# 959AI994/Multi-Gate-VAE

Measured on AMD Instinct MI355X. Metric: circuit-graphs/sec (train step), AIG-64k batch=64 per GPU, higher is better.
Workload: dtype f32 storage; dense products as bf16x3 split-precision MFMA, fp32 accumulate; 1 GPU; cfg2: DG_AE --type aig, 64 x 65536-node synthetic levelised DAGs per GPU (N=4194304, E=6558720, 120 levels), H=64, 4+4 rounds, layernorm, weights [1,4,4], negatives sampled; step includes the 7-scalar metrics copy (pinned, read one step behind); global_batch=64, parallelism=dp1

## Files before the change

### include/mgvae_hip.h

```cpp
#ifndef MGVAE_HIP_H
#define MGVAE_HIP_H
#include <stdint.h>
#ifdef __cplusplus
extern "C" {
#endif

#ifndef MGV_OK
#define MGV_OK 0
#define MGV_EINVAL (-1)
#define MGV_EUNSUPPORTED (-2)
#endif

int mgv_abi_version(void);

int mgv_struct_stage_fwd(int H, int64_t N, const float* h_in, const int32_t* nbr_ptr, const int32_t* nbr_idx,
                         const uint8_t* xcls, const float* xtab, int C, const float* Wc, const float* bc,
                         const float* Whh, const float* bhh, const float* ln_w, const float* ln_b, float ln_eps,
                         float* h_out, void* stream);
int mgv_struct_stage_bwd(int H, int64_t N, const float* h_in, const int32_t* nbr_ptr, const int32_t* nbr_idx,
                         const uint8_t* xcls, const float* xtab, int C, const float* Wc, const float* WcT,
                         const float* bc, const float* Whh, const float* WhhT, const float* bhh,
                         const float* ln_w, const float* ln_b, float ln_eps, const float* gy_direct,
                         const float* gy_agg, float* g_direct_out, float* g_agg_out, float* dWc, float* dbc,
                         float* dWhh, float* dbhh, float* dxtab, float* dln_w, float* dln_b, void* stream);
// ... 151 lines not shown
int mgv_cc_class_ws_ints(int64_t N);
int mgv_cc_class_count(int64_t N, const int32_t* label, int min_size, const int32_t* status, int32_t* ws, int64_t ws_ints, int32_t* counts,
                       void* stream);
int mgv_cc_class_fill(int64_t N, const int32_t* label, int64_t C, int64_t M, int32_t* ws, int64_t ws_ints, void* sort_temp,
                      int64_t sort_temp_ints, int64_t* class_ptr, int32_t* members, void* stream);
int mgv_sim_union(int H, int64_t N, const float* y, int ldy, const int32_t* graph_ptr, int G, float threshold, int32_t* parent,
                  int32_t* status, void* stream);
int mgv_recon_loss_fwd(int H, const float* s, const float* t, int ld, const int64_t* pos_src, const int64_t* pos_dst,
                       int64_t Epos, const int64_t* neg_src, const int64_t* neg_dst, int64_t Eneg,
                       double* sums, uint64_t* counts, int32_t* pred_bin, double* workspace, int64_t workspace_doubles,
                       void* stream);
int mgv_recon_loss_bwd(int H, int64_t N, const float* s, const float* t, int ld, const int64_t* pos_src, const int64_t* pos_dst,
                       int64_t Epos, const int32_t* pos_out_ptr, const int32_t* pos_out_dst, const int32_t* pos_in_ptr,
                       const int32_t* pos_in_src, const int64_t* neg_src, const int64_t* neg_dst, int64_t Eneg,
                       const float* gscale, float* ds, float* dt, void* stream);
int mgv_recon_loss_bwd_csr(int H, int64_t N, const float* s, const float* t, int ld, const int32_t* pos_out_ptr,
                           const int32_t* pos_out_dst, const int32_t* pos_in_ptr, const int32_t* pos_in_src, int64_t Epos,
                           const int32_t* neg_out_ptr, const int32_t* neg_out_dst, const int32_t* neg_in_ptr,
                           const int32_t* neg_in_src, int64_t Eneg, const float* gscale, float* ds, float* dt,
                           int skip_pos_longer_than , void* stream);
int mgv_recon_heavy_lists(int H, const float* s, const float* t, int ld, int64_t Epos, const float* gscale, int K,
                          const int32_t* nodes, const int32_t* node_seg_ptr, int S, const int32_t* seg_node, const int32_t* seg_e0,
                          const int32_t* seg_e1, const int32_t* list, int which, float* partial_ws, float* out, void* stream);
int mgv_link_keys(int H, const float* s, const float* t, int ld, const int64_t* pos_src, const int64_t* pos_dst, int64_t P,
                  const int64_t* neg_src, const int64_t* neg_dst, int64_t Q, uint32_t* keys, float* scores, int32_t* status,
                  void* stream);
int mgv_link_rank_work_ints(int64_t n);
int mgv_link_rank(int64_t n, int64_t P, const uint32_t* sorted_keys, const int32_t* order, double* out, int32_t* work,
                  int64_t work_ints, void* stream);
int mgv_neg_sample(int64_t N, int64_t E, uint64_t seed, const int32_t* pos_out_ptr, const int32_t* pos_out_dst,
                   int64_t* neg_src, int64_t* neg_dst, int32_t* cnt_out, int32_t* cnt_in, int32_t* rank_out, int32_t* rank_in,
                   void* stream);
int mgv_neg_bucket(int64_t E, const int64_t* neg_src, const int64_t* neg_dst, const int32_t* out_ptr, const int32_t* in_ptr,
                   const int32_t* rank_out, const int32_t* rank_in, int64_t* srt_src, int64_t* srt_dst, int32_t* out_dst, int32_t* in_src,
                   void* stream);

int mgv_func_loss_fwd(int H, int64_t P, const float* hf, const int64_t* pair_a, const int64_t* pair_b,
                      const float* tt, float eps, float* dis, double* ws, double* workspace, int64_t workspace_doubles,
                      void* stream);
int mgv_func_loss_bwd_csr(int H, int64_t N, int64_t P, const float* hf, const int64_t* pair_a, const int64_t* pair_b, const float* tt_sim,
                          const float* dis, float eps, const double* workspace8, const float* grad_loss, const int32_t* a_ptr,
                          const int32_t* a_pair, const int32_t* b_ptr, const int32_t* b_pair, const float* add, float* dhf, void* stream);
int mgv_func_loss_bwd(int H, int64_t P, const float* hf, const int64_t* pair_a, const int64_t* pair_b,
                      const float* tt, const float* dis, float eps, const double* ws, const float* gscale,
                      float* dhf, void* stream);

// ... 97 lines not shown
```

### multi-gate-vae_amd/csrc/losses.hip

```cpp
#include "mgv_common.h"
#include "mgv_slab.h"
#include "../../include/mgvae_hip.h"

namespace mgv {

__device__ __forceinline__ void atomic_add4(float* p, const float4& v) {
    atomicAdd(p + 0, v.x); atomicAdd(p + 1, v.y); atomicAdd(p + 2, v.z); atomicAdd(p + 3, v.w);
}

__device__ __forceinline__ double block_sum_d(double v, double* red) {
    const int tid = threadIdx.x;
    __syncthreads();
    red[tid] = v;
    __syncthreads();
    for (int s = kThreads / 2; s > 0; s >>= 1) {
        if (tid < s) red[tid] += red[tid + s];
        __syncthreads();
    }
    return red[0];
}

template <int H, bool BWD>
__global__ __launch_bounds__(kThreads) void k_edge_dot(int64_t E, const float* s, const float* t, int ld,
                                                       const int64_t* src, const int64_t* dst, int sigmoid,
                                                       float* out, const float* gout, float* ds, float* dt) {
    constexpr int LPR = H / 4, EPB = kThreads / LPR;
    const int lr = threadIdx.x % LPR, slot = threadIdx.x / LPR;
    for (int64_t e0 = (int64_t)blockIdx.x * EPB; e0 < E; e0 += (int64_t)gridDim.x * EPB) {
        const int64_t e = e0 + slot;
        const bool ok = e < E;
// ... 27 lines not shown
template <int H, bool BWD>
__global__ __launch_bounds__(kThreads) void k_recon(ReconArgs a) {
    constexpr int LPR = H / 4, EPB = kThreads / LPR;
    __shared__ double red[kThreads];
    const int lr = threadIdx.x % LPR, slot = threadIdx.x / LPR;
    const int64_t E = a.Ep + a.En;
    float lp = 0.f, ln = 0.f;
    unsigned int tp = 0, fp = 0, tn = 0, fn = 0;
    float g = 0.f;
    if (BWD) g = *a.gscale;
    const float wpos = BWD ? g / (float)a.Ep : 0.f, wneg = BWD ? g / (float)a.En : 0.f;
    for (int64_t e0 = (int64_t)blockIdx.x * EPB; e0 < E; e0 += (int64_t)gridDim.x * EPB) {
        const int64_t e = e0 + slot;
        const bool ok = e < E;
        const bool pos = e < a.Ep;
        float4 x = zero4(), y = zero4();
        int64_t u = 0, v = 0;
        if (ok) {
            u = pos ? a.psrc[e] : a.nsrc[e - a.Ep];
            v = pos ? a.pdst[e] : a.ndst[e - a.Ep];
            x = ld4(a.s + u * a.ld + 4 * lr);
            y = ld4(a.t + v * a.ld + 4 * lr);
        }
        const float val = group_sum<LPR>(dot4(x, y));
        const float p = sigmoidf_(val);
        if (!BWD) {
            if (ok && lr == 0) {
                const bool hit = p > 0.5f;
                if (pos) { lp -= logf(p + 1e-15f); tp += hit; fn += !hit; }
                else     { ln -= logf((1.0f - p) + 1e-15f); fp += hit; tn += !hit; }
                if (a.pred_bin) a.pred_bin[e] = hit ? 1 : 0;
            }
        } else if (ok) {
            const float dp = p * (1.0f - p);
            const float c = pos ? -wpos * dp / (p + 1e-15f) : wneg * dp / ((1.0f - p) + 1e-15f);
            atomic_add4(a.ds + u * a.ld + 4 * lr, scale4(c, y));
            atomic_add4(a.dt + v * a.ld + 4 * lr, scale4(c, x));
        }
    }
    if (!BWD) {
        const double sp = block_sum_d((double)lp, red);
        const double sn = block_sum_d((double)ln, red);
        const double c0 = block_sum_d((double)tp, red), c1 = block_sum_d((double)fp, red);
        const double c2 = block_sum_d((double)tn, red), c3 = block_sum_d((double)fn, red);
        if (threadIdx.x == 0) {
            a.slab[2 * blockIdx.x + 0] = sp; a.slab[2 * blockIdx.x + 1] = sn;
            atomicAdd(a.cnt + 0, (unsigned long long)c0); atomicAdd(a.cnt + 1, (unsigned long long)c1);
// ... 12 lines not shown
    const float w = -(*gscale) / (float)Ep;
    for (int64_t n0 = (int64_t)blockIdx.x * RPB; n0 < N; n0 += (int64_t)gridDim.x * RPB) {
        const int64_t u = n0 + slot;
        if (u >= N) continue;
        const float4 su = ld4(s + u * ld + 4 * lr), tu = ld4(t + u * ld + 4 * lr);
        float4 gs = zero4(), gt = zero4();
        for (int e = out_ptr[u]; e < out_ptr[u + 1]; ++e) {
            const float4 tv = ld4(t + (int64_t)out_dst[e] * ld + 4 * lr);
            const float p = sigmoidf_(group_sum<LPR>(dot4(su, tv)));
            gs = fma4(w * p * (1.0f - p) / (p + 1e-15f), tv, gs);
        }
        for (int e = in_ptr[u]; e < in_ptr[u + 1]; ++e) {
            const float4 sv = ld4(s + (int64_t)in_src[e] * ld + 4 * lr);
            const float p = sigmoidf_(group_sum<LPR>(dot4(sv, tu)));
            gt = fma4(w * p * (1.0f - p) / (p + 1e-15f), sv, gt);
        }
        float* pds = ds + u * ld + 4 * lr;
        float* pdt = dt + u * ld + 4 * lr;
        st4(pds, add4(ld4(pds), gs));
        st4(pdt, add4(ld4(pdt), gt));
    }
}

template <int H>
__global__ __launch_bounds__(kThreads) void k_recon_bwd_pull2(int64_t N, const float* s, const float* t, int ld,
                                                              const int32_t* pout_ptr, const int32_t* pout_dst, const int32_t* pin_ptr,
                                                              const int32_t* pin_src, int64_t Ep, const int32_t* nout_ptr,
                                                              const int32_t* nout_dst, const int32_t* nin_ptr, const int32_t* nin_src,
                                                              int64_t En, const float* gscale, float* ds, float* dt, int skip_len) {
    constexpr int LPR = H / 4, RPB = kThreads / LPR, K = 4;
    const int lr = threadIdx.x % LPR, slot = threadIdx.x / LPR;
    const float wp = Ep > 0 ? -(*gscale) / (float)Ep : 0.f, wn = En > 0 ? (*gscale) / (float)En : 0.f;
    int64_t first, end, stride;
    if ((gridDim.x & 7) == 0) {
        const int64_t chunk = ((N + 8 * RPB - 1) / (8 * RPB)) * RPB;
        first = (blockIdx.x & 7) * chunk + (int64_t)(blockIdx.x >> 3) * RPB;
        end = min(N, ((blockIdx.x & 7) + 1) * chunk);
        stride = (int64_t)(gridDim.x >> 3) * RPB;
    } else {
        first = (int64_t)blockIdx.x * RPB; end = N; stride = (int64_t)gridDim.x * RPB;
    }
    for (int64_t n0 = first; n0 < end; n0 += stride) {
        const int64_t u = n0 + slot;
        if (u >= end) continue;
        const float4 su = ld4(s + u * ld + 4 * lr), tu = ld4(t + u * ld + 4 * lr);
        int b0 = 0, b1 = 0, b2 = 0, b3 = 0, c0 = 0, c1 = 0, c2 = 0, c3 = 0;
        if (Ep > 0) {
            b0 = pout_ptr[u]; c0 = pout_ptr[u + 1] - b0;
            b1 = pin_ptr[u]; c1 = pin_ptr[u + 1] - b1;
            if (skip_len > 0 && c0 > skip_len) c0 = 0;
            if (skip_len > 0 && c1 > skip_len) c1 = 0;
        }
        if (En > 0) {
            b2 = nout_ptr[u]; c2 = nout_ptr[u + 1] - b2;
            b3 = nin_ptr[u]; c3 = nin_ptr[u + 1] - b3;
// ... 5 lines not shown
        float4 gs = zero4(), gt = zero4();
        int id[K];
#pragma unroll
        for (int k = 0; k < K; ++k) id[k] = k < c3 ? partner(k) : 0;
        for (int j0 = 0; j0 < c3; j0 += K) {
            float4 v[K];
#pragma unroll
            for (int k = 0; k < K; ++k) {
                const int j = j0 + k;
                const bool from_t = j < c0 || (j >= c1 && j < c2);
                if (j < c3) v[k] = ld4((from_t ? t : s) + (int64_t)id[k] * ld + 4 * lr);
            }
            int nid[K];
#pragma unroll
            for (int k = 0; k < K; ++k) nid[k] = j0 + K + k < c3 ? partner(j0 + K + k) : 0;
#pragma unroll
            for (int k = 0; k < K; ++k) {
                const int j = j0 + k;
                if (j < c3) {
                    const bool out = j < c0 || (j >= c1 && j < c2), pos = j < c1;
                    const float p = sigmoidf_(group_sum<LPR>(dot4(out ? su : tu, v[k])));
                    const float c = pos ? wp * p * (1.0f - p) / (p + 1e-15f) : wn * p * (1.0f - p) / ((1.0f - p) + 1e-15f);
                    if (out) gs = fma4(c, v[k], gs); else gt = fma4(c, v[k], gt);
                }
            }
#pragma unroll
            for (int k = 0; k < K; ++k) id[k] = nid[k];
        }
        st4(ds + u * ld + 4 * lr, gs);
        st4(dt + u * ld + 4 * lr, gt);
    }
}

template <int H>
__global__ __launch_bounds__(256) void k_recon_heavy_seg(int S, const int32_t* seg_node, const int32_t* seg_e0, const int32_t* seg_e1,
                                                         const int32_t* nodes, const float* s, const float* t, int ld, const int32_t* list,
                                                         int which, int64_t Ep, const float* gscale, float* partial) {
    constexpr int LPR = H / 4, G = 256 / LPR;
    __shared__ __attribute__((aligned(16))) float s_p[G][H];
    const int lr = threadIdx.x % LPR, grp = threadIdx.x / LPR;
    const float wp = -(*gscale) / (float)Ep;
    for (int sg = blockIdx.x; sg < S; sg += gridDim.x) {
        const int64_t u = nodes[seg_node[sg]];
        const float4 own = ld4((which ? t : s) + u * ld + 4 * lr);
        const float* other = which ? s : t;
        float4 acc = zero4();
        for (int e = seg_e0[sg] + grp; e < seg_e1[sg]; e += G) {
            const float4 v = ld4(other + (int64_t)list[e] * ld + 4 * lr);
            const float p = sigmoidf_(group_sum<LPR>(dot4(own, v)));
            acc = fma4(wp * p * (1.0f - p) / (p + 1e-15f), v, acc);
        }
        __syncthreads();
        st4(&s_p[grp][4 * lr], acc);
        __syncthreads();
        if (grp == 0) {
            float4 tot = zero4();
            for (int g = 0; g < G; ++g) tot = add4(tot, ld4(&s_p[g][4 * lr]));
            st4(partial + (int64_t)sg * H + 4 * lr, tot);
        }
    }
}

template <int H>
__global__ __launch_bounds__(kThreads) void k_recon_bwd_rows(int64_t E, const float* s, const float* t, int ld, const int64_t* src,
                                                             const int64_t* dst, int negative, float wscale, const float* gscale,
                                                             float* ds, float* dt) {
    constexpr int EPB = kThreads / H;
    const int l = threadIdx.x % H, slot = threadIdx.x / H;
    const float w = (*gscale) * wscale;
    for (int64_t e0 = (int64_t)blockIdx.x * EPB; e0 < E; e0 += (int64_t)gridDim.x * EPB) {
        const int64_t e = e0 + slot;
        const bool ok = e < E;
        int64_t u = 0, v = 0;
        float x = 0.f, y = 0.f;
        if (ok) { u = src[e]; v = dst[e]; x = s[u * ld + l]; y = t[v * ld + l]; }
        const float p = sigmoidf_(group_sum<H>(x * y));
        if (!ok) continue;
        const float dp = p * (1.0f - p);
        const float c = negative ? w * dp / ((1.0f - p) + 1e-15f) : -w * dp / (p + 1e-15f);
        atomicAdd(ds + u * ld + l, c * y);
        atomicAdd(dt + v * ld + l, c * x);
    }
}
// ... 254 lines not shown
        const int64_t* es = neg ? neg_src : pos_src;
        const int64_t* ed = neg ? neg_dst : pos_dst;
        const float wsc = 1.0f / (float)E;
        switch (H) {
            case 16: hipLaunchKernelGGL((mgv::k_recon_bwd_rows<16>), dim3(mgv::items_grid(E, mgv::kThreads / 16)), dim3(mgv::kThreads), 0, st, E, s, t, ld, es, ed, neg, wsc, gscale, ds, dt); break;
            case 32: hipLaunchKernelGGL((mgv::k_recon_bwd_rows<32>), dim3(mgv::items_grid(E, mgv::kThreads / 32)), dim3(mgv::kThreads), 0, st, E, s, t, ld, es, ed, neg, wsc, gscale, ds, dt); break;
            case 64: hipLaunchKernelGGL((mgv::k_recon_bwd_rows<64>), dim3(mgv::items_grid(E, mgv::kThreads / 64)), dim3(mgv::kThreads), 0, st, E, s, t, ld, es, ed, neg, wsc, gscale, ds, dt); break;
            default: return MGV_EUNSUPPORTED;
        }
    }
    MGV_LAUNCH_RET();
}

extern "C" int mgv_recon_loss_bwd_csr(int H, int64_t N, const float* s, const float* t, int ld, const int32_t* pos_out_ptr,
                                      const int32_t* pos_out_dst, const int32_t* pos_in_ptr, const int32_t* pos_in_src, int64_t Epos,
                                      const int32_t* neg_out_ptr, const int32_t* neg_out_dst, const int32_t* neg_in_ptr,
                                      const int32_t* neg_in_src, int64_t Eneg, const float* gscale, float* ds, float* dt,
                                      int skip_pos_longer_than, void* stream) {
    MGV_CHECK_ARG(s && t && gscale && ds && dt && Epos >= 0 && Eneg >= 0 && N >= 0 && ld >= H && ld % 4 == 0 && skip_pos_longer_than >= 0);
    MGV_CHECK_ARG(Epos == 0 || (pos_out_ptr && pos_out_dst && pos_in_ptr && pos_in_src));
    MGV_CHECK_ARG(Eneg == 0 || (neg_out_ptr && neg_out_dst && neg_in_ptr && neg_in_src));
    if (N == 0) return MGV_OK;
    hipStream_t st = static_cast<hipStream_t>(stream);
    MGV_DISPATCH_H(H, hipLaunchKernelGGL((mgv::k_recon_bwd_pull2<HH>), dim3(mgv::items_grid(N, mgv::kThreads / (HH / 4))), dim3(mgv::kThreads), 0, st,
                                         N, s, t, ld, pos_out_ptr, pos_out_dst, pos_in_ptr, pos_in_src, Epos, neg_out_ptr, neg_out_dst,
                                         neg_in_ptr, neg_in_src, Eneg, gscale, ds, dt, skip_pos_longer_than));
    MGV_LAUNCH_RET();
}

extern "C" int mgv_recon_heavy_lists(int H, const float* s, const float* t, int ld, int64_t Epos, const float* gscale, int K,
                                     const int32_t* nodes, const int32_t* node_seg_ptr, int S, const int32_t* seg_node, const int32_t* seg_e0,
                                     const int32_t* seg_e1, const int32_t* list, int which, float* partial_ws, float* out, void* stream) {
    MGV_CHECK_ARG(K >= 0 && S >= 0 && Epos > 0 && s && t && gscale && out && ld >= H && ld % 4 == 0 && (which == 0 || which == 1));
    if (K == 0 || S == 0) return MGV_OK;
    MGV_CHECK_ARG(nodes && node_seg_ptr && seg_node && seg_e0 && seg_e1 && list && partial_ws);
    hipStream_t st = static_cast<hipStream_t>(stream);
    MGV_DISPATCH_H(H, hipLaunchKernelGGL((mgv::k_recon_heavy_seg<HH>), dim3(S < 4096 ? S : 4096), dim3(256), 0, st, S, seg_node, seg_e0, seg_e1, nodes,
                                         s, t, ld, list, which, Epos, gscale, partial_ws));
    hipLaunchKernelGGL(mgv::k_heavy_add, dim3((K + 15) / 16 < 1024 ? (K + 15) / 16 : 1024), dim3(256), 0, st, K, H, nodes, node_seg_ptr, partial_ws, out, ld, 1);
    MGV_LAUNCH_RET();
}

extern "C" int mgv_func_loss_fwd(int H, int64_t P, const float* hf, const int64_t* pair_a, const int64_t* pair_b,
                                 const float* tt, float eps, float* dis, double* ws, double* workspace, int64_t workspace_doubles,
                                 void* stream) {
    MGV_CHECK_ARG(P >= 2 && hf && pair_a && pair_b && tt && dis && ws);
    hipStream_t st = static_cast<hipStream_t>(stream);
    int g1 = 0;
    MGV_DISPATCH_H(H, g1 = mgv::items_grid(P, mgv::kThreads / (HH / 4)));
    const int g2 = mgv::items_grid(P, mgv::kThreads);
    MGV_CHECK_ARG(workspace && workspace_doubles >= 4 * (int64_t)g1 && workspace_doubles >= 3 * (int64_t)g2);
    MGV_DISPATCH_H(H, hipLaunchKernelGGL((mgv::k_func_dist<HH>), dim3(g1), dim3(mgv::kThreads), 0, st, P, hf, pair_a, pair_b, tt, eps, dis, workspace));
    mgv::launch_slab_sum<double, double>(workspace, g1, 4, 4, ws, st);
    hipLaunchKernelGGL(mgv::k_func_l1, dim3(g2), dim3(mgv::kThreads), 0, st, P, dis, tt, ws, workspace);
    mgv::launch_slab_sum<double, double>(workspace, g2, 3, 3, ws + 4, st);
    MGV_LAUNCH_RET();
}

extern "C" int mgv_func_loss_bwd_csr(int H, int64_t N, int64_t P, const float* hf, const int64_t* pair_a, const int64_t* pair_b, const float* tt,
                                     const float* dis, float eps, const double* ws, const float* gscale, const int32_t* a_ptr,
                                     const int32_t* a_pair, const int32_t* b_ptr, const int32_t* b_pair, const float* add, float* dhf, void* stream) {
    MGV_CHECK_ARG(N >= 0 && P >= 2 && hf && pair_a && pair_b && tt && dis && ws && gscale && a_ptr && a_pair && b_ptr && b_pair && dhf);
// ... 52 lines not shown
```

### multi-gate-vae_amd/deepgate/_model_base.py

```python
import os

import torch
from torch import nn

from . import ops
from .arch.mlp import MLP
from .arch.tfmlp import TFMlpAggr
from .data import plan_of
from .digae_layer import DirectedInnerProductDecoder
from .sampling import NegativeEdges, negative_sampling, negative_sampling_device

EPS = 1e-15
DEVICE_SAMPLER = True
MAX_LOGSTD = 10


class FunctionalModel(nn.Module):
    ENCODER_ATTR = 'struct_encoder'
    GATES = ()

    def __init__(self, struct_encoder, num_rounds=1, dim_hidden=128, enable_encode=True, enable_reverse=True):
        super().__init__()
        setattr(self, self.ENCODER_ATTR, struct_encoder)
        self.decoder = DirectedInnerProductDecoder()
# ... 100 lines not shown
        with torch.no_grad():
            s, t = self._decoder_halves(hs)
            return ops.reconstruct_edges(s, t, graph_ptr=graph_ptr, threshold=threshold, skip_self=skip_self, by=by,
                                         with_scores=with_scores, max_edges=max_edges)

    def similar_gates(self, hf, k, graph_ptr=None, threshold=0.999):
        return ops.sim_topk(hf, k, graph_ptr=graph_ptr, threshold=threshold)

    def equivalence_candidates(self, hf, graph_ptr=None, threshold=0.999, with_scores=False, max_pairs=None):
        return ops.sim_pairs(hf, graph_ptr=graph_ptr, threshold=threshold, with_scores=with_scores, max_pairs=max_pairs)

    def equivalence_classes(self, hf, graph_ptr=None, threshold=0.999, min_size=2):
        return ops.sim_classes(hf, graph_ptr=graph_ptr, threshold=threshold, min_size=min_size)

    def similarity_profile(self, hf, thresholds, graph_ptr=None):
        return ops.counts_above(ops.sim_profile(hf, thresholds, graph_ptr=graph_ptr))

    def equivalence_threshold(self, hf, max_pairs, graph_ptr=None, lo=0.0):
        return ops.sim_threshold_for(hf, max_pairs, graph_ptr=graph_ptr, lo=lo)

    def functional_similarity(self, hf, pair_index):
        return ops.sim_at(hf, pair_index)

    def recon_loss(self, hs, pos_edge_index, neg_edge_index=None, want_pred=True, edge_keys=None, plan=None, pass_hs=False, want_rank=False):
        if pass_hs and hs.requires_grad:
            st, self._hs_pass = ops.linear_passthrough(hs, self.hs_decompose.weight, self.hs_decompose.bias)
        else:
            st = ops.linear(hs, self.hs_decompose.weight, self.hs_decompose.bias)
        if plan is not None and (plan.E != pos_edge_index.shape[1] or plan.N != hs.shape[0]):
            plan = None
        neg_csr = None
        if neg_edge_index is None:
            neg_edge_index = self._draw_negatives(hs, pos_edge_index, plan, edge_keys)
        if plan is not None and hs.is_cuda and torch.is_tensor(neg_edge_index) and neg_edge_index.shape[1] > 0:
            cache = getattr(plan, '_neg_cache', None)
            key = (neg_edge_index.data_ptr(), neg_edge_index._version, tuple(neg_edge_index.shape), hs.shape[0])
            if cache is None or cache[0] is not neg_edge_index or cache[1] != key:
                from .sampling import bucket_negatives
                cache = plan._neg_cache = (neg_edge_index, key, bucket_negatives(neg_edge_index.long(), hs.shape[0]))
            neg_edge_index = cache[2]
        if isinstance(neg_edge_index, NegativeEdges):
            neg_csr, neg_edge_index = neg_edge_index.csr, neg_edge_index.edge_index
        loss, counts, pred_bin = ops.ReconLossFn.apply(st, pos_edge_index, neg_edge_index, want_pred, plan, neg_csr)
        self.last_confusion = counts
        self.last_link_metrics = ops.link_record(st, None, pos_edge_index, neg_edge_index) if want_rank else None
        Ep, En = pos_edge_index.shape[1], neg_edge_index.shape[1]
        gt_bin = None
        if want_pred:
            gt_bin = torch.zeros(Ep + En, dtype=torch.int32, device=hs.device)
            gt_bin[:Ep] = 1
        return loss, pred_bin if want_pred else None, gt_bin

    def load(self, model_path):
        checkpoint = torch.load(model_path, map_location=lambda storage, loc: storage)
        src = checkpoint['state_dict']
        state = {}
        for k, v in src.items():
            state[k[7:] if k.startswith('module') and not k.startswith('module_list') else k] = v
        own = self.state_dict()
        for k in list(state):
            if k in own:
                if state[k].shape != own[k].shape:
                    print('Skip loading parameter {}, required shape{}, loaded shape{}.'.format(k, own[k].shape, state[k].shape))
                    state[k] = own[k]
            else:
                print('Drop parameter {}.'.format(k))
# ... 11 lines not shown
```

### multi-gate-vae_amd/deepgate/ops.py

```python
from collections import namedtuple

import torch

from . import _hip
from ._hip import HipLibraryError, check, ptr

import os

F32 = torch.float32
I32 = torch.int32
U8 = torch.uint8
LN_EPS = 1e-5

PRECISION = os.environ.get('MGV_PRECISION', 'x3')
FIRST_STAGE_TABLE = True


def use_x3(H):
    return PRECISION == 'x3' and H in (32, 64)


def split_bf16(w):
    hi = w.to(torch.bfloat16)
    lo = (w - hi.to(torch.float32)).to(torch.bfloat16)
    return hi, lo


def frag_order(w):
    R, K = w.shape
    return w.reshape(R // 16, 16, K // 32, 4, 8).permute(0, 2, 3, 1, 4).reshape(-1)
# ... 1360 lines not shown

def sim_classes(x, graph_ptr=None, threshold=SIM_THRESHOLD, min_size=2, route='walk', eps=1e-8, max_pairs=None):
    if route not in ('walk', 'pairs'):
        raise HipLibraryError("sim_classes: route must be 'walk' (classes straight from the tile walk) or 'pairs' (sim_pairs, then "
                              "components), got %r" % (route,))
    min_size = _min_size(min_size)
    if route == 'walk' and max_pairs is not None:
        raise HipLibraryError("sim_classes: max_pairs belongs to route='pairs'; the walk holds no pair list")
    if route == 'pairs':
        pi, _, _ = sim_pairs(x, graph_ptr=graph_ptr, threshold=threshold, max_pairs=max_pairs, eps=eps)
        with torch.no_grad():
            label, status = _cc_from_pairs(pi, x.shape[0])
            return (label,) + _class_table(label, min_size, status, 'sim_classes')
    y = row_unit(x, eps)
    with torch.no_grad():
        N, H = y.shape
        gp, G = _pair_graphs(graph_ptr, y.device)
        parent, status = _cc_forest(N, y.device)
        _hip.call('mgv_sim_union', H, N, ptr(y), H, ptr(gp), G, float(threshold), ptr(parent), ptr(status))
        label = _cc_labels(N, parent)
        return (label,) + _class_table(label, min_size, status, 'sim_classes')


class ReconLossFn(torch.autograd.Function):

    @staticmethod
    def forward(ctx, st, pos_edge_index, neg_edge_index, want_pred, plan=None, neg_csr=None):
        std = check(st.detach().contiguous(), F32, 'st')
        N, H2 = std.shape
        H = H2 // 2
        ps, pd = _edge_rows(pos_edge_index)
        ns, nd = _edge_rows(neg_edge_index)
        Ep, En = ps.numel(), ns.numel()
        dev = std.device
        sums = torch.zeros(2, dtype=torch.float64, device=dev)
        counts = torch.zeros(4, dtype=torch.int64, device=dev)
        pred = torch.empty(Ep + En, dtype=torch.int32, device=dev) if want_pred else None
        t_view = std[:, H:]
        _hip.call('mgv_recon_loss_fwd', H, ptr(std), ptr(t_view), H2, ptr(ps), ptr(pd), Ep, ptr(ns), ptr(nd), En,
                  ptr(sums), ptr(counts), ptr(pred), *_sw(std.device))
        loss = (sums[0] / max(Ep, 1) + sums[1] / max(En, 1)).to(F32)
        ctx.save_for_backward(std, ps, pd, ns, nd)
        ctx.plan, ctx.neg_csr = plan, neg_csr
        ctx.mark_non_differentiable(counts)
        if pred is not None:
            ctx.mark_non_differentiable(pred)
            return loss, counts, pred
        return loss, counts, torch.empty(0, dtype=torch.int32, device=dev)

    @staticmethod
    def backward(ctx, gloss, _gc, _gp):
        global _SWEEP_BWD_EVENT
        if _SWEEP_BWD_EVENT is not None and gloss.is_cuda:
            torch.cuda.current_stream().wait_event(_SWEEP_BWD_EVENT)
            _SWEEP_BWD_EVENT = None
        std, ps, pd, ns, nd = ctx.saved_tensors
        H2 = std.shape[1]
        H = H2 // 2
        g = gloss.detach().to(F32).reshape(1).contiguous()
        pl = ctx.plan
        if pl is not None and ctx.neg_csr is not None:
            dst_ = torch.empty_like(std)
            heavy = [(0, pl.heavy_segments(True), pl.out_dst), (1, pl.heavy_segments(False), pl.in_src)]
            skip = pl.HEAVY_ROW if any(hv is not None for _, hv, _ in heavy) else 0
            _hip.call('mgv_recon_loss_bwd_csr', H, std.shape[0], ptr(std), ptr(std[:, H:]), H2, ptr(pl.out_ptr), ptr(pl.out_dst),
                      ptr(pl.in_ptr), ptr(pl.in_src), ps.numel(), *[ptr(c) for c in ctx.neg_csr], ns.numel(), ptr(g), ptr(dst_),
                      ptr(dst_[:, H:]), skip)
            for which, hv, lst in heavy:
                if hv is not None:
                    pw = workspace(hv['S'] * H, std.device)
                    _hip.call('mgv_recon_heavy_lists', H, ptr(std), ptr(std[:, H:]), H2, ps.numel(), ptr(g), hv['K'], ptr(hv['nodes']),
                              ptr(hv['node_seg_ptr']), hv['S'], ptr(hv['seg_node']), ptr(hv['seg_e0']), ptr(hv['seg_e1']), ptr(lst), which,
                              ptr(pw), ptr(dst_[:, H:]) if which else ptr(dst_))
            return dst_, None, None, None, None, None
        dst_ = torch.zeros_like(std)
        csr = (pl.out_ptr, pl.out_dst, pl.in_ptr, pl.in_src) if pl is not None else (None, None, None, None)
        _hip.call('mgv_recon_loss_bwd', H, std.shape[0], ptr(std), ptr(std[:, H:]), H2, ptr(ps), ptr(pd), ps.numel(),
                  *[ptr(c) for c in csr], ptr(ns), ptr(nd), ns.numel(), ptr(g), ptr(dst_), ptr(dst_[:, H:]))
        return dst_, None, None, None, None, None


def confusion_counts(pred_bin, gt_bin):
    counts = torch.zeros(4, dtype=torch.int64, device=pred_bin.device)
    _hip.call('mgv_confusion', pred_bin.numel(), ptr(check(pred_bin.contiguous(), torch.int32, 'pred_bin')),
              ptr(check(gt_bin.contiguous(), torch.int32, 'gt_bin')), ptr(counts))
    return counts


LINK_RECORD_WORDS = 8


def link_record(st_or_s, t=None, pos_edge_index=None, neg_edge_index=None, return_scores=False):
    neg = getattr(neg_edge_index, 'edge_index', neg_edge_index)
    P, Q = int(pos_edge_index.shape[1]), int(neg.shape[1])
    if P == 0 or Q == 0:
        raise ValueError('Only one class present (%d positive, %d negative pairs): ROC-AUC and average precision are not defined' % (P, Q))
    sd = check(st_or_s.detach().contiguous(), F32, 'st' if t is None else 's')
    if t is None:
        ld = sd.shape[1]
        H = ld // 2
        td = sd[:, H:]
    else:
# ... 293 lines not shown
```

### multi-gate-vae_amd/deepgate/trainer.py

```python
import inspect
import os
import sys
import time

import numpy as np
import torch
from torch import nn

from . import ops
from .data import CircuitBatch
from .optim import FlatAdam
from .prefetch import BatchPrefetcher
from .sampling import sorted_edge_keys
from .synthetic import collate as collate_arrays
from .utils.logger import Logger
from .utils.model_utils import load_model
from .utils.utils import AverageMeter


class GraphLoader:

    def __init__(self, graphs, batch_size, shuffle, rank=0, world_size=1, seed=0):
        self.graphs, self.batch_size, self.shuffle = graphs, batch_size, shuffle
        self.rank, self.world_size, self.seed, self.epoch = rank, world_size, seed, 0
# ... 106 lines not shown
        checkpoint = torch.load(path, map_location='cpu')
        self.optimizer.load_state_dict(checkpoint['optimizer'])
        for param_group in self.optimizer.param_groups:
            self.lr = param_group['lr']
        self.model_epoch = checkpoint['epoch']
        self.model.load(path)
        print('[INFO] Continue training from epoch {:}'.format(self.model_epoch))
        return path

    def resume(self):
        model_path = os.path.join(self.log_dir, 'model_last.pth')
        if os.path.exists(model_path):
            self.model, self.optimizer, self.model_epoch = load_model(self.model, model_path, optimizer=self.optimizer,
                                                                      local_rank=self.local_rank, device=self.device)
            return True
        return False

    def run_batch(self, batch, want_pred=True, want_rank=False):
        batch.train_pos_edge_index = batch.edge_index
        neg = getattr(batch, 'neg_edge_index', None)
        dev_is_cuda = next(self.model.parameters()).is_cuda
        if getattr(self, '_has_after_hs', None) is None:
            self._has_after_hs = 'after_hs' in inspect.signature(self.model.forward).parameters
        side = self._side_stream() if (self.overlap and dev_is_cuda and self._has_after_hs) else None

        def recon(hs, pass_hs=False):
            k = None
            if neg is None and getattr(batch, '_mgv_plan', None) is None:
                k = getattr(batch, '_mgv_edge_keys', None)
                if k is None:
                    k = batch._mgv_edge_keys = sorted_edge_keys(batch.edge_index, batch.num_nodes)
            return self.model.recon_loss(hs, batch.train_pos_edge_index, neg, want_pred=want_pred, edge_keys=k,
                                         plan=getattr(batch, '_mgv_plan', None), **({'pass_hs': True} if pass_hs else {}),
                                         **({'want_rank': True} if want_rank else {}))

        def recon_on_side(hs):
            side.wait_event(self.model._hs_ready)
            hs.record_stream(side)
            with torch.cuda.stream(side):
                return recon(hs, pass_hs=True)

        if side is not None:
            hs, hf = self.model(batch, after_hs=recon_on_side)
            loss, pred_bin, gt_bin = self.model.after_hs_out
            self.model.after_hs_out = None
            main = torch.cuda.current_stream()
            main.wait_stream(side)
            for t in (loss, pred_bin, gt_bin, self.model.last_confusion, self.model.last_link_metrics if want_rank else None):
                if t is not None:
                    t.record_stream(main)
        else:
            hs, hf = self.model(batch)
            loss, pred_bin, gt_bin = recon(hs)
        loss_status = {'recon_loss': loss, 'pred_bin': pred_bin, 'gt_bin': gt_bin}
        if 'VAE' in getattr(self.args, 'model', '') and hasattr(self.model, 'kl_loss'):
            s_kl, t_kl = self.model.kl_loss()
            loss_status['kl_loss'] = s_kl + t_kl
# ... 131 lines not shown
```

Measured before the change: 1007 graphs/s.

## Fuse recon loss forward into backward CSR pull pass with expected grad scale

When a CSR plan and negative CSR are available and predictions are not needed, the recon loss forward now runs the backward pull kernel. It computes the gradient rows using the expected loss weight while also accumulating loss sums and confusion counts, so the separate edge-wise forward pass and the later backward pass become one pass over the edges. In backward, a small kernel rescales the precomputed gradient only if the actual upstream gradient differs from the expected scale. This trades an extra stored N×2H gradient buffer and a redundant non-contracted dot per edge for removing one full edge traversal.

Measured after the change: 1022 graphs/s (median of 6 runs). +1.5%, better.

```diff
diff --git a/include/mgvae_hip.h b/include/mgvae_hip.h
--- a/include/mgvae_hip.h
+++ b/include/mgvae_hip.h
@@ -197,6 +197,17 @@
 int mgv_recon_heavy_lists(int H, const float* s, const float* t, int ld, int64_t Epos, const float* gscale, int K,
                           const int32_t* nodes, const int32_t* node_seg_ptr, int S, const int32_t* seg_node, const int32_t* seg_e0,
                           const int32_t* seg_e1, const int32_t* list, int which, float* partial_ws, float* out, void* stream);
+int mgv_recon_step_csr(int H, int64_t N, const float* s, const float* t, int ld, const int32_t* pos_out_ptr,
+                       const int32_t* pos_out_dst, const int32_t* pos_in_ptr, const int32_t* pos_in_src, int64_t Epos,
+                       const int32_t* neg_out_ptr, const int32_t* neg_out_dst, const int32_t* neg_in_ptr,
+                       const int32_t* neg_in_src, int64_t Eneg, float expect_scale, double* sums, uint64_t* counts, float* ds,
+                       float* dt, int skip_pos_longer_than, double* workspace, int64_t workspace_doubles, void* stream);
+int mgv_recon_step_heavy_lists(int H, const float* s, const float* t, int ld, int64_t Epos, float expect_scale, int K,
+                               const int32_t* nodes, const int32_t* node_seg_ptr, int S, const int32_t* seg_node,
+                               const int32_t* seg_e0, const int32_t* seg_e1, const int32_t* list, int which, float* partial_ws,
+                               float* out, double* sums, uint64_t* counts, double* workspace, int64_t workspace_doubles,
+                               void* stream);
+int mgv_rows_rescale_unless(int64_t n_floats, float* rows, const float* g_dev, float expect_scale, void* stream);
 int mgv_link_keys(int H, const float* s, const float* t, int ld, const int64_t* pos_src, const int64_t* pos_dst, int64_t P,
                   const int64_t* neg_src, const int64_t* neg_dst, int64_t Q, uint32_t* keys, float* scores, int32_t* status,
                   void* stream);
diff --git a/multi-gate-vae_amd/csrc/losses.hip b/multi-gate-vae_amd/csrc/losses.hip
--- a/multi-gate-vae_amd/csrc/losses.hip
+++ b/multi-gate-vae_amd/csrc/losses.hip
@@ -6,6 +6,16 @@
 
 __device__ __forceinline__ void atomic_add4(float* p, const float4& v) {
     atomicAdd(p + 0, v.x); atomicAdd(p + 1, v.y); atomicAdd(p + 2, v.z); atomicAdd(p + 3, v.w);
+}
+
+__device__ __forceinline__ float dot4_plain(const float4& a, const float4& b) {
+#pragma clang fp contract(off)
+    return a.x * b.x + a.y * b.y + a.z * b.z + a.w * b.w;
+}
+
+__device__ __forceinline__ float4 opaque4(float4 v) {
+    asm("" : "+v"(v.x), "+v"(v.y), "+v"(v.z), "+v"(v.w));
+    return v;
 }
 
 __device__ __forceinline__ double block_sum_d(double v, double* red) {
@@ -79,7 +89,7 @@
             x = ld4(a.s + u * a.ld + 4 * lr);
             y = ld4(a.t + v * a.ld + 4 * lr);
         }
-        const float val = group_sum<LPR>(dot4(x, y));
+        const float val = group_sum<LPR>(dot4_plain(x, y));
         const float p = sigmoidf_(val);
         if (!BWD) {
             if (ok && lr == 0) {
@@ -138,15 +148,19 @@
     }
 }
 
-template <int H>
+template <int H, bool STEP>
 __global__ __launch_bounds__(kThreads) void k_recon_bwd_pull2(int64_t N, const float* s, const float* t, int ld,
                                                               const int32_t* pout_ptr, const int32_t* pout_dst, const int32_t* pin_ptr,
                                                               const int32_t* pin_src, int64_t Ep, const int32_t* nout_ptr,
                                                               const int32_t* nout_dst, const int32_t* nin_ptr, const int32_t* nin_src,
-                                                              int64_t En, const float* gscale, float* ds, float* dt, int skip_len) {
+                                                              int64_t En, const float* gscale, float gval, float* ds, float* dt, int skip_len,
+                                                              double* slab, unsigned long long* cnt) {
     constexpr int LPR = H / 4, RPB = kThreads / LPR, K = 4;
     const int lr = threadIdx.x % LPR, slot = threadIdx.x / LPR;
-    const float wp = Ep > 0 ? -(*gscale) / (float)Ep : 0.f, wn = En > 0 ? (*gscale) / (float)En : 0.f;
+    const float g = STEP ? gval : *gscale;
+    const float wp = Ep > 0 ? -g / (float)Ep : 0.f, wn = En > 0 ? g / (float)En : 0.f;
+    double lp = 0, ln = 0;
+    unsigned int tp = 0, fp = 0, tn = 0, fn = 0;
     int64_t first, end, stride;
     if ((gridDim.x & 7) == 0) {
         const int64_t chunk = ((N + 8 * RPB - 1) / (8 * RPB)) * RPB;
@@ -198,6 +212,14 @@
                     const float p = sigmoidf_(group_sum<LPR>(dot4(out ? su : tu, v[k])));
                     const float c = pos ? wp * p * (1.0f - p) / (p + 1e-15f) : wn * p * (1.0f - p) / ((1.0f - p) + 1e-15f);
                     if (out) gs = fma4(c, v[k], gs); else gt = fma4(c, v[k], gt);
+                    if (STEP && out) {
+                        const float q = sigmoidf_(group_sum<LPR>(dot4_plain(opaque4(su), v[k])));
+                        const bool hit = q > 0.5f;
+                        if (lr == 0) {
+                            if (pos) { lp -= (double)logf(q + 1e-15f); tp += hit; fn += !hit; }
+                            else     { ln -= (double)logf((1.0f - q) + 1e-15f); fp += hit; tn += !hit; }
+                        }
+                    }
                 }
             }
 #pragma unroll
@@ -206,16 +228,31 @@
         st4(ds + u * ld + 4 * lr, gs);
         st4(dt + u * ld + 4 * lr, gt);
     }
-}
-
-template <int H>
+    if (STEP) {
+        __shared__ double red[kThreads];
+        const double sp = block_sum_d(lp, red), sn = block_sum_d(ln, red);
+        const double c0 = block_sum_d((double)tp, red), c1 = block_sum_d((double)fp, red);
+        const double c2 = block_sum_d((double)tn, red), c3 = block_sum_d((double)fn, red);
+        if (threadIdx.x == 0) {
+            slab[2 * blockIdx.x + 0] = sp; slab[2 * blockIdx.x + 1] = sn;
+            atomicAdd(cnt + 0, (unsigned long long)c0); atomicAdd(cnt + 1, (unsigned long long)c1);
+            atomicAdd(cnt + 2, (unsigned long long)c2); atomicAdd(cnt + 3, (unsigned long long)c3);
+        }
+    }
+}
+
+template <int H, bool STEP>
 __global__ __launch_bounds__(256) void k_recon_heavy_seg(int S, const int32_t* seg_node, const int32_t* seg_e0, const int32_t* seg_e1,
                                                          const int32_t* nodes, const float* s, const float* t, int ld, const int32_t* list,
-                                                         int which, int64_t Ep, const float* gscale, float* partial) {
+                                                         int which, int64_t Ep, const float* gscale, float gval, float* partial,
+                                                         double* slab, unsigned long long* cnt) {
     constexpr int LPR = H / 4, G = 256 / LPR;
+    static_assert(kThreads == 256, "block_sum_d reduces kThreads values");
     __shared__ __attribute__((aligned(16))) float s_p[G][H];
     const int lr = threadIdx.x % LPR, grp = threadIdx.x / LPR;
-    const float wp = -(*gscale) / (float)Ep;
+    const float wp = -(STEP ? gval : *gscale) / (float)Ep;
+    double lp = 0;
+    unsigned int tp = 0, fn = 0;
     for (int sg = blockIdx.x; sg < S; sg += gridDim.x) {
         const int64_t u = nodes[seg_node[sg]];
         const float4 own = ld4((which ? t : s) + u * ld + 4 * lr);
@@ -225,6 +262,11 @@
             const float4 v = ld4(other + (int64_t)list[e] * ld + 4 * lr);
             const float p = sigmoidf_(group_sum<LPR>(dot4(own, v)));
             acc = fma4(wp * p * (1.0f - p) / (p + 1e-15f), v, acc);
+            if (STEP && which == 0) {
+                const float q = sigmoidf_(group_sum<LPR>(dot4_plain(opaque4(own), v)));
+                const bool hit = q > 0.5f;
+                if (lr == 0) { lp -= (double)logf(q + 1e-15f); tp += hit; fn += !hit; }
+            }
         }
         __syncthreads();
         st4(&s_p[grp][4 * lr], acc);
@@ -235,6 +277,25 @@
             st4(partial + (int64_t)sg * H + 4 * lr, tot);
         }
     }
+    if (STEP && which == 0) {
+        __shared__ double red[kThreads];
+        const double sp = block_sum_d(lp, red);
+        const double c0 = block_sum_d((double)tp, red), c3 = block_sum_d((double)fn, red);
+        if (threadIdx.x == 0) {
+            slab[blockIdx.x] = sp;
+            atomicAdd(cnt + 0, (unsigned long long)c0); atomicAdd(cnt + 3, (unsigned long long)c3);
+        }
+    }
+}
+
+__global__ __launch_bounds__(kThreads) void k_rows_rescale_unless(int64_t n, float* rows, const float* g_dev, float expect) {
+    const float g = *g_dev;
+    if (g == expect) return;
+    const float f = g / expect;
+    const int64_t n4 = n / 4;
+    for (int64_t i = (int64_t)blockIdx.x * kThreads + threadIdx.x; i < n4; i += (int64_t)gridDim.x * kThreads)
+        st4(rows + 4 * i, scale4(f, ld4(rows + 4 * i)));
+    if (blockIdx.x == 0 && threadIdx.x < n - 4 * n4) rows[4 * n4 + threadIdx.x] *= f;
 }
 
 template <int H>
@@ -535,9 +596,30 @@
     MGV_CHECK_ARG(Eneg == 0 || (neg_out_ptr && neg_out_dst && neg_in_ptr && neg_in_src));
     if (N == 0) return MGV_OK;
     hipStream_t st = static_cast<hipStream_t>(stream);
-    MGV_DISPATCH_H(H, hipLaunchKernelGGL((mgv::k_recon_bwd_pull2<HH>), dim3(mgv::items_grid(N, mgv::kThreads / (HH / 4))), dim3(mgv::kThreads), 0, st,
+    MGV_DISPATCH_H(H, hipLaunchKernelGGL((mgv::k_recon_bwd_pull2<HH, false>), dim3(mgv::items_grid(N, mgv::kThreads / (HH / 4))), dim3(mgv::kThreads), 0, st,
                                          N, s, t, ld, pos_out_ptr, pos_out_dst, pos_in_ptr, pos_in_src, Epos, neg_out_ptr, neg_out_dst,
-                                         neg_in_ptr, neg_in_src, Eneg, gscale, ds, dt, skip_pos_longer_than));
+                                         neg_in_ptr, neg_in_src, Eneg, gscale, 0.f, ds, dt, skip_pos_longer_than, nullptr, nullptr));
+    MGV_LAUNCH_RET();
+}
+
+extern "C" int mgv_recon_step_csr(int H, int64_t N, const float* s, const float* t, int ld, const int32_t* pos_out_ptr,
+                                  const int32_t* pos_out_dst, const int32_t* pos_in_ptr, const int32_t* pos_in_src, int64_t Epos,
+                                  const int32_t* neg_out_ptr, const int32_t* neg_out_dst, const int32_t* neg_in_ptr,
+                                  const int32_t* neg_in_src, int64_t Eneg, float expect_scale, double* sums, uint64_t* counts, float* ds,
+                                  float* dt, int skip_pos_longer_than, double* workspace, int64_t workspace_doubles, void* stream) {
+    MGV_CHECK_ARG(s && t && sums && counts && ds && dt && Epos >= 0 && Eneg >= 0 && N >= 0 && ld >= H && ld % 4 == 0 && skip_pos_longer_than >= 0);
+    MGV_CHECK_ARG(Epos == 0 || (pos_out_ptr && pos_out_dst && pos_in_ptr && pos_in_src));
+    MGV_CHECK_ARG(Eneg == 0 || (neg_out_ptr && neg_out_dst && neg_in_ptr && neg_in_src));
+    if (N == 0) return MGV_OK;
+    hipStream_t st = static_cast<hipStream_t>(stream);
+    int grid = 0;
+    MGV_DISPATCH_H(H, grid = mgv::items_grid(N, mgv::kThreads / (HH / 4)));
+    MGV_CHECK_ARG(workspace && workspace_doubles >= 2 * (int64_t)grid);
+    MGV_DISPATCH_H(H, hipLaunchKernelGGL((mgv::k_recon_bwd_pull2<HH, true>), dim3(grid), dim3(mgv::kThreads), 0, st,
+                                         N, s, t, ld, pos_out_ptr, pos_out_dst, pos_in_ptr, pos_in_src, Epos, neg_out_ptr, neg_out_dst,
+                                         neg_in_ptr, neg_in_src, Eneg, nullptr, expect_scale, ds, dt, skip_pos_longer_than, workspace,
+                                         reinterpret_cast<unsigned long long*>(counts)));
+    mgv::launch_slab_sum<double, double>(workspace, grid, 2, 2, sums, st);
     MGV_LAUNCH_RET();
 }
 
@@ -548,9 +630,38 @@
     if (K == 0 || S == 0) return MGV_OK;
     MGV_CHECK_ARG(nodes && node_seg_ptr && seg_node && seg_e0 && seg_e1 && list && partial_ws);
     hipStream_t st = static_cast<hipStream_t>(stream);
-    MGV_DISPATCH_H(H, hipLaunchKernelGGL((mgv::k_recon_heavy_seg<HH>), dim3(S < 4096 ? S : 4096), dim3(256), 0, st, S, seg_node, seg_e0, seg_e1, nodes,
-                                         s, t, ld, list, which, Epos, gscale, partial_ws));
+    MGV_DISPATCH_H(H, hipLaunchKernelGGL((mgv::k_recon_heavy_seg<HH, false>), dim3(S < 4096 ? S : 4096), dim3(256), 0, st, S, seg_node, seg_e0, seg_e1, nodes,
+                                         s, t, ld, list, which, Epos, gscale, 0.f, partial_ws, nullptr, nullptr));
     hipLaunchKernelGGL(mgv::k_heavy_add, dim3((K + 15) / 16 < 1024 ? (K + 15) / 16 : 1024), dim3(256), 0, st, K, H, nodes, node_seg_ptr, partial_ws, out, ld, 1);
+    MGV_LAUNCH_RET();
+}
+
+extern "C" int mgv_recon_step_heavy_lists(int H, const float* s, const float* t, int ld, int64_t Epos, float expect_scale, int K,
+                                          const int32_t* nodes, const int32_t* node_seg_ptr, int S, const int32_t* seg_node,
+                                          const int32_t* seg_e0, const int32_t* seg_e1, const int32_t* list, int which, float* partial_ws,
+                                          float* out, double* sums, uint64_t* counts, double* workspace, int64_t workspace_doubles,
+                                          void* stream) {
+    MGV_CHECK_ARG(K >= 0 && S >= 0 && Epos > 0 && s && t && out && ld >= H && ld % 4 == 0 && (which == 0 || which == 1));
+    MGV_CHECK_ARG(which == 1 || (sums && counts));
+    if (K == 0 || S == 0) return MGV_OK;
+    MGV_CHECK_ARG(nodes && node_seg_ptr && seg_node && seg_e0 && seg_e1 && list && partial_ws);
+    const int grid = S < 4096 ? S : 4096;
+    MGV_CHECK_ARG(which == 1 || (workspace && workspace_doubles >= (int64_t)grid));
+    hipStream_t st = static_cast<hipStream_t>(stream);
+    MGV_DISPATCH_H(H, hipLaunchKernelGGL((mgv::k_recon_heavy_seg<HH, true>), dim3(grid), dim3(256), 0, st, S, seg_node, seg_e0, seg_e1, nodes,
+                                         s, t, ld, list, which, Epos, nullptr, expect_scale, partial_ws, workspace,
+                                         reinterpret_cast<unsigned long long*>(counts)));
+    if (which == 0) mgv::launch_slab_sum<double, double>(workspace, grid, 1, 1, sums, st);
+    hipLaunchKernelGGL(mgv::k_heavy_add, dim3((K + 15) / 16 < 1024 ? (K + 15) / 16 : 1024), dim3(256), 0, st, K, H, nodes, node_seg_ptr, partial_ws, out, ld, 1);
+    MGV_LAUNCH_RET();
+}
+
+extern "C" int mgv_rows_rescale_unless(int64_t n_floats, float* rows, const float* g_dev, float expect_scale, void* stream) {
+    MGV_CHECK_ARG(n_floats >= 0 && g_dev && expect_scale != 0.f && expect_scale == expect_scale);
+    if (n_floats == 0) return MGV_OK;
+    MGV_CHECK_ARG(rows && (reinterpret_cast<uintptr_t>(rows) & 15) == 0);
+    hipLaunchKernelGGL(mgv::k_rows_rescale_unless, dim3(mgv::items_grid(n_floats, 4 * mgv::kThreads)), dim3(mgv::kThreads), 0,
+                       static_cast<hipStream_t>(stream), n_floats, rows, g_dev, expect_scale);
     MGV_LAUNCH_RET();
 }
 
diff --git a/multi-gate-vae_amd/deepgate/_model_base.py b/multi-gate-vae_amd/deepgate/_model_base.py
--- a/multi-gate-vae_amd/deepgate/_model_base.py
+++ b/multi-gate-vae_amd/deepgate/_model_base.py
@@ -146,7 +146,8 @@
     def functional_similarity(self, hf, pair_index):
         return ops.sim_at(hf, pair_index)
 
-    def recon_loss(self, hs, pos_edge_index, neg_edge_index=None, want_pred=True, edge_keys=None, plan=None, pass_hs=False, want_rank=False):
+    def recon_loss(self, hs, pos_edge_index, neg_edge_index=None, want_pred=True, edge_keys=None, plan=None, pass_hs=False, want_rank=False,
+                   expect_scale=1.0):
         if pass_hs and hs.requires_grad:
             st, self._hs_pass = ops.linear_passthrough(hs, self.hs_decompose.weight, self.hs_decompose.bias)
         else:
@@ -165,7 +166,7 @@
             neg_edge_index = cache[2]
         if isinstance(neg_edge_index, NegativeEdges):
             neg_csr, neg_edge_index = neg_edge_index.csr, neg_edge_index.edge_index
-        loss, counts, pred_bin = ops.ReconLossFn.apply(st, pos_edge_index, neg_edge_index, want_pred, plan, neg_csr)
+        loss, counts, pred_bin = ops.ReconLossFn.apply(st, pos_edge_index, neg_edge_index, want_pred, plan, neg_csr, expect_scale)
         self.last_confusion = counts
         self.last_link_metrics = ops.link_record(st, None, pos_edge_index, neg_edge_index) if want_rank else None
         Ep, En = pos_edge_index.shape[1], neg_edge_index.shape[1]
diff --git a/multi-gate-vae_amd/deepgate/ops.py b/multi-gate-vae_amd/deepgate/ops.py
--- a/multi-gate-vae_amd/deepgate/ops.py
+++ b/multi-gate-vae_amd/deepgate/ops.py
@@ -1,11 +1,11 @@
 from collections import namedtuple
+import math
+import os
 
 import torch
 
 from . import _hip
 from ._hip import HipLibraryError, check, ptr
-
-import os
 
 F32 = torch.float32
 I32 = torch.int32
@@ -1412,10 +1412,23 @@
         return (label,) + _class_table(label, min_size, status, 'sim_classes')
 
 
+def _recon_heavy(plan):
+    heavy = [(0, plan.heavy_segments(True), plan.out_dst), (1, plan.heavy_segments(False), plan.in_src)]
+    return heavy, (plan.HEAVY_ROW if any(hv is not None for _, hv, _ in heavy) else 0)
+
+
 class ReconLossFn(torch.autograd.Function):
 
-    @staticmethod
-    def forward(ctx, st, pos_edge_index, neg_edge_index, want_pred, plan=None, neg_csr=None):
+    @classmethod
+    def apply(cls, st, pos_edge_index, neg_edge_index, want_pred, plan=None, neg_csr=None, expect_scale=1.0):
+        expect_scale = float(expect_scale)
+        one_pass = bool(plan is not None and neg_csr is not None and not want_pred and torch.is_grad_enabled() and st.requires_grad
+                        and st.is_cuda and expect_scale != 0.0 and math.isfinite(expect_scale)
+                        and os.environ.get('MGV_RECON_ONE_PASS', '1') != '0')
+        return super().apply(st, pos_edge_index, neg_edge_index, want_pred, plan, neg_csr, expect_scale if one_pass else None)
+
+    @staticmethod
+    def forward(ctx, st, pos_edge_index, neg_edge_index, want_pred, plan=None, neg_csr=None, expect_scale=None):
         std = check(st.detach().contiguous(), F32, 'st')
         N, H2 = std.shape
         H = H2 // 2
@@ -1427,8 +1440,23 @@
         counts = torch.zeros(4, dtype=torch.int64, device=dev)
         pred = torch.empty(Ep + En, dtype=torch.int32, device=dev) if want_pred else None
         t_view = std[:, H:]
-        _hip.call('mgv_recon_loss_fwd', H, ptr(std), ptr(t_view), H2, ptr(ps), ptr(pd), Ep, ptr(ns), ptr(nd), En,
-                  ptr(sums), ptr(counts), ptr(pred), *_sw(std.device))
+        ctx.dst_ = ctx.expect_scale = None
+        if expect_scale is not None:
+            dst_ = torch.empty_like(std)
+            heavy, skip = _recon_heavy(plan)
+            _hip.call('mgv_recon_step_csr', H, N, ptr(std), ptr(t_view), H2, ptr(plan.out_ptr), ptr(plan.out_dst), ptr(plan.in_ptr),
+                      ptr(plan.in_src), Ep, *[ptr(c) for c in neg_csr], En, expect_scale, ptr(sums), ptr(counts), ptr(dst_),
+                      ptr(dst_[:, H:]), skip, *_sw(dev))
+            for which, hv, lst in heavy:
+                if hv is not None:
+                    pw = workspace(hv['S'] * H, dev)
+                    _hip.call('mgv_recon_step_heavy_lists', H, ptr(std), ptr(t_view), H2, Ep, expect_scale, hv['K'], ptr(hv['nodes']),
+                              ptr(hv['node_seg_ptr']), hv['S'], ptr(hv['seg_node']), ptr(hv['seg_e0']), ptr(hv['seg_e1']), ptr(lst), which,
+                              ptr(pw), ptr(dst_[:, H:]) if which else ptr(dst_), ptr(sums), ptr(counts), *_sw(dev))
+            ctx.dst_, ctx.expect_scale = dst_, expect_scale
+        else:
+            _hip.call('mgv_recon_loss_fwd', H, ptr(std), ptr(t_view), H2, ptr(ps), ptr(pd), Ep, ptr(ns), ptr(nd), En,
+                      ptr(sums), ptr(counts), ptr(pred), *_sw(std.device))
         loss = (sums[0] / max(Ep, 1) + sums[1] / max(En, 1)).to(F32)
         ctx.save_for_backward(std, ps, pd, ns, nd)
         ctx.plan, ctx.neg_csr = plan, neg_csr
@@ -1449,10 +1477,13 @@
         H = H2 // 2
         g = gloss.detach().to(F32).reshape(1).contiguous()
         pl = ctx.plan
+        if ctx.dst_ is not None:
+            dst_, ctx.dst_ = ctx.dst_, None
+            _hip.call('mgv_rows_rescale_unless', dst_.numel(), ptr(dst_), ptr(g), ctx.expect_scale)
+            return dst_, None, None, None, None, None, None
         if pl is not None and ctx.neg_csr is not None:
             dst_ = torch.empty_like(std)
-            heavy = [(0, pl.heavy_segments(True), pl.out_dst), (1, pl.heavy_segments(False), pl.in_src)]
-            skip = pl.HEAVY_ROW if any(hv is not None for _, hv, _ in heavy) else 0
+            heavy, skip = _recon_heavy(pl)
             _hip.call('mgv_recon_loss_bwd_csr', H, std.shape[0], ptr(std), ptr(std[:, H:]), H2, ptr(pl.out_ptr), ptr(pl.out_dst),
                       ptr(pl.in_ptr), ptr(pl.in_src), ps.numel(), *[ptr(c) for c in ctx.neg_csr], ns.numel(), ptr(g), ptr(dst_),
                       ptr(dst_[:, H:]), skip)
@@ -1462,12 +1493,12 @@
                     _hip.call('mgv_recon_heavy_lists', H, ptr(std), ptr(std[:, H:]), H2, ps.numel(), ptr(g), hv['K'], ptr(hv['nodes']),
                               ptr(hv['node_seg_ptr']), hv['S'], ptr(hv['seg_node']), ptr(hv['seg_e0']), ptr(hv['seg_e1']), ptr(lst), which,
                               ptr(pw), ptr(dst_[:, H:]) if which else ptr(dst_))
-            return dst_, None, None, None, None, None
+            return dst_, None, None, None, None, None, None
         dst_ = torch.zeros_like(std)
         csr = (pl.out_ptr, pl.out_dst, pl.in_ptr, pl.in_src) if pl is not None else (None, None, None, None)
         _hip.call('mgv_recon_loss_bwd', H, std.shape[0], ptr(std), ptr(std[:, H:]), H2, ptr(ps), ptr(pd), ps.numel(),
                   *[ptr(c) for c in csr], ptr(ns), ptr(nd), ns.numel(), ptr(g), ptr(dst_), ptr(dst_[:, H:]))
-        return dst_, None, None, None, None, None
+        return dst_, None, None, None, None, None, None
 
 
 def confusion_counts(pred_bin, gt_bin):
diff --git a/multi-gate-vae_amd/deepgate/trainer.py b/multi-gate-vae_amd/deepgate/trainer.py
--- a/multi-gate-vae_amd/deepgate/trainer.py
+++ b/multi-gate-vae_amd/deepgate/trainer.py
@@ -152,6 +152,7 @@
         dev_is_cuda = next(self.model.parameters()).is_cuda
         if getattr(self, '_has_after_hs', None) is None:
             self._has_after_hs = 'after_hs' in inspect.signature(self.model.forward).parameters
+            self._has_expect_scale = 'expect_scale' in inspect.signature(self.model.recon_loss).parameters
         side = self._side_stream() if (self.overlap and dev_is_cuda and self._has_after_hs) else None
 
         def recon(hs, pass_hs=False):
@@ -162,7 +163,8 @@
                     k = batch._mgv_edge_keys = sorted_edge_keys(batch.edge_index, batch.num_nodes)
             return self.model.recon_loss(hs, batch.train_pos_edge_index, neg, want_pred=want_pred, edge_keys=k,
                                          plan=getattr(batch, '_mgv_plan', None), **({'pass_hs': True} if pass_hs else {}),
-                                         **({'want_rank': True} if want_rank else {}))
+                                         **({'want_rank': True} if want_rank else {}),
+                                         **({'expect_scale': self.rc_prob_func_weight[0]} if self._has_expect_scale else {}))
 
         def recon_on_side(hs):
             side.wait_event(self.model._hs_ready)
```
